# bupt-ai-cz/HIAST

Hardware: AMD Instinct MI355X
Metric: self-training images/sec (fwd+bwd+pseudo-label) at 1024x512 (higher is better)
Workload: dtype fp16

## Files before the change

### hiast_amd/csrc/conv_launch.h

```cpp
#pragma once
#include <stdlib.h>

#include "common.h"

namespace hiast {

struct IGeo {
    int H, W, Ho, Wo, stride, dil;
};

}

struct ConvLaunch {
    const void* x = nullptr;
    const void* wp = nullptr;
    void* y = nullptr;
    const void* res = nullptr;
    const void* res_gate = nullptr;
    int gate_mask = 0;
    const float* gamma = nullptr;
    const float* beta = nullptr;
    const float* mean = nullptr;
    const float* var = nullptr;
    float eps = 0.0f;
    int relu = 0;
    int64_t M = 0;
    int K = 0, N = 0, taps = 1;
    hiast::IGeo geo = {0, 0, 0, 0, 1, 1};
    int fmt = HIAST_FMT_BF16;
    int out_f32 = 0;
    float* stats = nullptr;
    int stats_rows = 0;
    int stats_mode = 0;
    hipStream_t st = nullptr;

    int planes() const { return hiast_fmt_planes(fmt); }
    bool f16() const { return fmt == HIAST_FMT_FP16; }
};

enum class ConvFamily { XCONV, XCONV2, TILE_F16, TILE };

struct ConvRoute {
    ConvFamily family = ConvFamily::TILE;
    int BN = 0, BM = 0;
    bool half9 = false;
    int rows = 0;
};

static inline int conv_panel_streams(int64_t M, int NG, int panel_rows)
{
    static const int env_cus = [] { const char* e = getenv("HIAST_XCONV_CUS"); const int v = e ? atoi(e) : 0; return v >= 8 && v <= 256 ? v : 0; }();
    const long long npanel = (M + panel_rows - 1) / panel_rows;
    long long streams = (env_cus ? env_cus : hiast_grid_cus()) / NG / 8 * 8;
    if (streams < 8) streams = 8;
    if (streams > npanel) streams = (npanel + 7) / 8 * 8;
    return (int)streams;
}

ConvRoute ig_route(const ConvLaunch& c);
int hiast_igemm_launch(const ConvLaunch& c);
int hiast_igemm_launch_f16(const ConvLaunch& c, const ConvRoute& r);
int hiast_xconv_ok(const ConvLaunch& c);
int hiast_xconv_stats_rows(int64_t M, int N);
int hiast_xconv_launch(const ConvLaunch& c, const ConvRoute& r);
int hiast_xconv2_ok(const ConvLaunch& c);
int hiast_xconv2_launch(const ConvLaunch& c);
int hiast_gemm_nt_launch(const void* x, const float* w, void* y, int64_t M, int K, int N, int dtype, hipStream_t st);
```

### hiast_amd/csrc/igemm.hip

```cpp
#include "igemm_kernel.h"

namespace hiast {

template <int PL>
__device__ __forceinline__ size_t ig_wp_elem(int n, int t, int k, int taps, int KO)
{
    const size_t row = ((size_t)n * taps + t) * PL * KO;
    return PL == 2 ? row + (size_t)(k >> 5) * 64 + (k & 31) : row + k;
}

template <int PL, bool F16 = false>
__global__ __launch_bounds__(256) void pack_conv_weight_kernel(const float* __restrict__ w,
                                                               unsigned short* __restrict__ wp,
                                                               unsigned short* __restrict__ wpt, int N, int K, int taps,
                                                               int mode)
{
    const long long idx = (long long)blockIdx.x * 256 + threadIdx.x;
    if (idx >= (long long)N * taps * K) return;
    const int k = (int)(idx % K);
    const int t = (int)((idx / K) % taps);
    const int n = (int)(idx / ((long long)K * taps));
    const float v = w[((size_t)n * K + k) * taps + t];
    unsigned short h, l = 0;
    if (F16) h = H16<true>::enc(v);
    else ig_split(v, h, l);
    if (mode != 1) {
        unsigned short* d = wp + ig_wp_elem<PL>(n, t, k, taps, K);
        d[0] = h;
        if (PL == 2) d[32] = l;
    }
    if (mode != 0) {
        unsigned short* d = (mode == 1 ? wp : wpt) + ig_wp_elem<PL>(k, taps - 1 - t, n, taps, N);
        d[0] = h;
        if (PL == 2) d[32] = l;
    }
}

constexpr int PK_PITCH = 72;

template <int PL, bool F16 = false>
__device__ __forceinline__ void pack_tile(const float* __restrict__ w, unsigned short* __restrict__ wp,
                                          unsigned short* __restrict__ wpt, int N, int K, int taps, int mode, int n0,
                                          int k0, unsigned short* lds)
{
    constexpr int TN = PL == 1 ? 32 : 16;
    unsigned short* hi = lds;
    unsigned short* lo = lds + (PL == 2 ? TN * taps * PK_PITCH : 0);
    unsigned short* fwd = (mode == 1) ? nullptr : wp;
    unsigned short* adj = (mode == 0) ? nullptr : (mode == 1 ? wp : wpt);
    const int run = 64 * taps;
    for (int nh = 0; nh < 64; nh += TN) {
        if (nh) __syncthreads();
        for (int e = threadIdx.x; e < TN * run; e += 256) {
            const int n = e / run, r = e - n * run;
            const int k = r / taps, t = r - k * taps;
            const float v = w[((size_t)(n0 + nh + n) * K + k0) * taps + r];
            unsigned short h, l = 0;
            if (F16) h = H16<true>::enc(v);
            else ig_split(v, h, l);
            hi[(n * taps + t) * PK_PITCH + k] = h;
            if (PL == 2) lo[(n * taps + t) * PK_PITCH + k] = l;
        }
        __syncthreads();
        if (fwd) {
            for (int e = threadIdx.x; e < TN * taps * 8; e += 256) {
                const int c = e & 7, nt = e >> 3;
                const int n = nt / taps, t = nt - n * taps;
                const uint4 vh = *reinterpret_cast<const uint4*>(&hi[nt * PK_PITCH + c * 8]);
                unsigned short* d = fwd + ig_wp_elem<PL>(n0 + nh + n, t, k0 + c * 8, taps, K);
                *reinterpret_cast<uint4*>(d) = vh;
                if (PL == 2) *reinterpret_cast<uint4*>(d + 32) = *reinterpret_cast<const uint4*>(&lo[nt * PK_PITCH + c * 8]);
            }
        }
        if (adj) {
            for (int e = threadIdx.x; e < 64 * taps * (TN / 8); e += 256) {
                const int c = e % (TN / 8), kt = e / (TN / 8);
                const int k = kt / taps, t = kt - k * taps;
                unsigned short vh[8], vl[8];
#pragma unroll
                for (int j = 0; j < 8; ++j) {
                    vh[j] = hi[((c * 8 + j) * taps + t) * PK_PITCH + k];
                    if (PL == 2) vl[j] = lo[((c * 8 + j) * taps + t) * PK_PITCH + k];
                }
                unsigned short* d = adj + ig_wp_elem<PL>(k0 + k, taps - 1 - t, n0 + nh + c * 8, taps, N);
                *reinterpret_cast<uint4*>(d) = make_uint4(vh[0] | (unsigned)vh[1] << 16, vh[2] | (unsigned)vh[3] << 16,
                                                          vh[4] | (unsigned)vh[5] << 16, vh[6] | (unsigned)vh[7] << 16);
                if (PL == 2)
                    *reinterpret_cast<uint4*>(d + 32) = make_uint4(vl[0] | (unsigned)vl[1] << 16, vl[2] | (unsigned)vl[3] << 16,
                                                                   vl[4] | (unsigned)vl[5] << 16, vl[6] | (unsigned)vl[7] << 16);
            }
        }
    }
}

template <int PL, bool F16 = false>
__global__ __launch_bounds__(256) void pack_conv_weight_tiled_kernel(const float* __restrict__ w,
                                                                     unsigned short* __restrict__ wp,
                                                                     unsigned short* __restrict__ wpt, int N, int K,
                                                                     int taps, int mode)
{
    extern __shared__ __attribute__((aligned(16))) unsigned short lds[];
    const int kt = K / 64;
    pack_tile<PL, F16>(w, wp, wpt, N, K, taps, mode, (int)(blockIdx.x / kt) * 64, (int)(blockIdx.x % kt) * 64, lds);
}

__global__ __launch_bounds__(256) void pack_conv_weight_multi_kernel(const hiast_pack_rec* __restrict__ table,
                                                                     const int32_t* __restrict__ chunk_tensor,
                                                                     const int64_t* __restrict__ chunk_start)
{
    extern __shared__ __attribute__((aligned(16))) unsigned short lds[];
    const hiast_pack_rec r = table[chunk_tensor[blockIdx.x]];
    const int kt = r.K / 64;
    const int tile = (int)chunk_start[blockIdx.x];
    const int n0 = (tile / kt) * 64, k0 = (tile % kt) * 64;
    if (r.planes == HIAST_FMT_SPLIT_BF16)
        pack_tile<2>(r.w, (unsigned short*)r.wp, (unsigned short*)r.wpt, r.N, r.K, r.taps, r.mode, n0, k0, lds);
    else if (r.planes == HIAST_FMT_FP16)
        pack_tile<1, true>(r.w, (unsigned short*)r.wp, (unsigned short*)r.wpt, r.N, r.K, r.taps, r.mode, n0, k0, lds);
    else
        pack_tile<1>(r.w, (unsigned short*)r.wp, (unsigned short*)r.wpt, r.N, r.K, r.taps, r.mode, n0, k0, lds);
}

__global__ __launch_bounds__(256) void to_planes_kernel(const float* __restrict__ x, unsigned short* __restrict__ p,
                                                        long long M, int C)
{
    const long long total8 = M * C / 8;
    for (long long i = (long long)blockIdx.x * 256 + threadIdx.x; i < total8; i += (long long)gridDim.x * 256) {
        const long long m = (i * 8) / C;
        const int c = (int)((i * 8) - m * C);
        const float4 a = reinterpret_cast<const float4*>(x)[2 * i], b = reinterpret_cast<const float4*>(x)[2 * i + 1];
        const float v[8] = {a.x, a.y, a.z, a.w, b.x, b.y, b.z, b.w};
        unsigned ph[4], pl_[4];
#pragma unroll
        for (int q = 0; q < 4; ++q) {
            unsigned short h0, l0, h1, l1;
            ig_split(v[2 * q], h0, l0);
            ig_split(v[2 * q + 1], h1, l1);
            ph[q] = (unsigned)h0 | ((unsigned)h1 << 16);
            pl_[q] = (unsigned)l0 | ((unsigned)l1 << 16);
        }
        unsigned short* dst = p + ig_elem<2>((size_t)m, c, C);
        *reinterpret_cast<uint4*>(dst) = make_uint4(ph[0], ph[1], ph[2], ph[3]);
        *reinterpret_cast<uint4*>(dst + 32) = make_uint4(pl_[0], pl_[1], pl_[2], pl_[3]);
    }
}

__global__ __launch_bounds__(256) void from_planes_kernel(const unsigned short* __restrict__ p, float* __restrict__ x,
                                                          long long M, int C)
{
    const long long total8 = M * C / 8;
    for (long long i = (long long)blockIdx.x * 256 + threadIdx.x; i < total8; i += (long long)gridDim.x * 256) {
        const long long m = (i * 8) / C;
        const int c = (int)((i * 8) - m * C);
        const unsigned short* src = p + ig_elem<2>((size_t)m, c, C);
        const uint4 h = *reinterpret_cast<const uint4*>(src), l = *reinterpret_cast<const uint4*>(src + 32);
        const unsigned wh[4] = {h.x, h.y, h.z, h.w}, wl[4] = {l.x, l.y, l.z, l.w};
        float v[8];
#pragma unroll
        for (int q = 0; q < 4; ++q) {
            v[2 * q] = __uint_as_float(wh[q] << 16) + __uint_as_float(wl[q] << 16);
            v[2 * q + 1] = __uint_as_float(wh[q] & 0xFFFF0000u) + __uint_as_float(wl[q] & 0xFFFF0000u);
        }
        reinterpret_cast<float4*>(x)[2 * i] = make_float4(v[0], v[1], v[2], v[3]);
        reinterpret_cast<float4*>(x)[2 * i + 1] = make_float4(v[4], v[5], v[6], v[7]);
    }
}

}

struct IgEnv {
    int half;
    int bn;
    int ragged_off;
    int cosched0;
};
static const IgEnv& ig_env()
{
    static const IgEnv env = [] {
        IgEnv e;
        const char* v = getenv("HIAST_IGEMM_HALF");
        e.half = v ? (atoi(v) != 0) : -1;
        v = getenv("HIAST_IGEMM_BN");
        const int bn = v ? atoi(v) : 0;
        e.bn = (bn == 64 || bn == 128 || bn == 256) ? bn : 0;
        e.ragged_off = getenv("HIAST_IGEMM_RAGGED") != nullptr;
        v = getenv("HIAST_IGEMM_COSCHED");
        e.cosched0 = v && atoi(v) != 0;
        return e;
    }();
    return env;
}
static thread_local int ig_cosched_tls = -1, ig_half_tls = -1;
extern "C" int hiast_igemm_set_half(int v)
{
    const int prev = ig_half_tls;
    ig_half_tls = v < 0 ? -1 : (v != 0);
    return prev;
}
extern "C" int hiast_igemm_set_cosched(int on)
{
    const int prev = ig_cosched_tls;
    ig_cosched_tls = on < 0 ? -1 : (on != 0);
    return prev;
}
static int ig_half_forced() { return ig_half_tls >= 0 ? ig_half_tls : ig_env().half; }
static int ig_cosched() { return ig_cosched_tls >= 0 ? ig_cosched_tls : ig_env().cosched0; }

#ifndef IG_HALF_AUTO
#define IG_HALF_BLOCKS(M, N) ((((M) + 255) / 256) * (((N) % 256 == 0) ? (N) / 256 : (N) / 128))
#define IG_HALF_AUTO(M, K, N) (IG_HALF_BLOCKS(M, N) <= 64 || (IG_HALF_BLOCKS(M, N) <= 128 && !ig_cosched()))
#endif
static int ig_half_tile(int64_t M, int K, int N, int taps, int out_f32)
{
    if (taps != 1 || out_f32 || N % 128 != 0 || M < 4096) return 0;
    if (ig_half_forced() >= 0) return ig_half_forced();
    return IG_HALF_AUTO(M, K, N);
}
static int ig_half_tile9(int64_t M, int N, int PL, bool bn_relu_only)
{
    if (PL != 2 || !bn_relu_only || N % 128 != 0 || M < 4096) return 0;
    if (ig_half_forced() >= 0) return ig_half_forced();
    return IG_HALF_AUTO(M, 0, N);
}

ConvRoute ig_route(const ConvLaunch& c)
{
    ConvRoute r;
    if (c.stats_mode != 2 && hiast_xconv_ok(c)) {
        r.family = ConvFamily::XCONV;
        r.rows = hiast_xconv_stats_rows(c.M, c.N);
        return r;
    }
    if (c.stats_mode == 0 && !c.f16() && hiast_xconv2_ok(c)) {
        r.family = ConvFamily::XCONV2;
        return r;
    }
    r.family = c.f16() ? ConvFamily::TILE_F16 : ConvFamily::TILE;
    r.BN = (c.N % 256 == 0) ? 256 : ((c.N % 128 == 0) ? 128 : 64);
    const bool plain = !c.mean && !c.gamma && !c.res && !c.relu && !c.res_gate && c.stats_mode == 0;
    if (plain && !c.out_f32 && r.BN == 128 && c.N > 512 && !ig_env().ragged_off) r.BN = 256;
    if (const int v = ig_env().bn) {
        if (c.N % v == 0) r.BN = v;
    }
    r.half9 = c.taps == 9 && !c.out_f32 && c.geo.stride == 1 &&
              ig_half_tile9(c.M, c.N, c.planes(), c.mean && c.relu && !c.res && !c.res_gate && c.stats_mode == 0) != 0;
    const bool half = r.half9 || (c.geo.stride >= 0 && ig_half_tile(c.M, c.K, c.N, c.taps, c.out_f32) != 0);
    if (half) r.BN = 128;
    r.BM = half ? 128 : hiast::IG_BM;
    r.rows = (int)((c.M + r.BM - 1) / r.BM);
    return r;
}

int hiast_igemm_launch(const ConvLaunch& in)
{
    ConvLaunch c = in;
    if (c.stats_mode != 2) c.stats_mode = c.stats ? 1 : 0;
    const int H = c.geo.H, W = c.geo.W, stride = c.geo.stride, dil = c.geo.dil;
    if (!hiast_fmt_ok(c.fmt)) return HIAST_E_RANGE;
    const int planes = c.planes();
    if (c.stats_mode == 2) {
        if (!c.stats || !c.res || !c.mean || !c.var || planes != 1 || c.out_f32 || c.relu || c.res_gate || c.N % 8) return HIAST_E_RANGE;
    } else {
        if (c.stats && (planes != 1 || c.out_f32 || c.res || c.relu)) return HIAST_E_RANGE;
        if ((c.stats || c.res_gate) && c.mean) return HIAST_E_RANGE;
    }
    if (c.res_gate && (planes != 1 || !c.res || c.relu || c.out_f32 || (!c.gate_mask && (((uintptr_t)c.res_gate) & 15)))) return HIAST_E_RANGE;
    if (!c.x || !c.wp || !c.y || (c.mean && !c.var)) return HIAST_E_ARG;
    if (c.M <= 0 || c.K <= 0 || c.N <= 0) return HIAST_E_ARG;
    if ((planes != 1 && planes != 2) || (c.taps != 1 && c.taps != 9)) return HIAST_E_RANGE;
    if ((c.K * planes) % 64 != 0 || c.N % 64 != 0 || c.M > (1ll << 31) - 512) return HIAST_E_RANGE;
    if (c.out_f32 && c.res) return HIAST_E_RANGE;
    if ((((uintptr_t)c.x) | ((uintptr_t)c.wp) | ((uintptr_t)c.y) | ((uintptr_t)c.res)) & 15) return HIAST_E_RANGE;
    c.geo = {0, 0, 0, 0, 1, 1};
    size_t in_pix = (size_t)c.M;
    if (c.taps != 1 && stride == -2) {
        if (H <= 0 || W <= 0 || dil != 1 || planes != 1 || c.out_f32) return HIAST_E_ARG;
        const int Hs = (H - 1) / 2 + 1, Ws = (W - 1) / 2 + 1;
        if (c.M % ((int64_t)H * W) != 0) return HIAST_E_ARG;
        c.geo = {Hs, Ws, H, W, -2, 1};
        in_pix = (size_t)(c.M / ((int64_t)H * W)) * Hs * Ws;
    } else if (c.taps != 1) {
        if (H <= 0 || W <= 0 || stride <= 0 || dil <= 0) return HIAST_E_ARG;
        const int Ho = (H - 1) / stride + 1, Wo = (W - 1) / stride + 1;
        if (c.M % ((int64_t)Ho * Wo) != 0) return HIAST_E_ARG;
        c.geo = {H, W, Ho, Wo, stride, dil};
        in_pix = (size_t)(c.M / ((int64_t)Ho * Wo)) * H * W;
    }
    if (in_pix * planes * c.K * 2 >= (1ull << 31) || (size_t)c.N * c.taps * planes * c.K * 2 >= (1ull << 31)) return HIAST_E_RANGE;
    const ConvRoute r = ig_route(c);
    if (c.stats_mode != 0 && c.stats_rows != r.rows) return HIAST_E_ARG;
    switch (r.family) {
    case ConvFamily::XCONV: return hiast_xconv_launch(c, r);
    case ConvFamily::XCONV2: return hiast_xconv2_launch(c);
    case ConvFamily::TILE_F16: return hiast_igemm_launch_f16(c, r);
    case ConvFamily::TILE: break;
    }
    if (planes == 2) return c.out_f32 ? launch_igemm_t<2, true>(c, r) : launch_igemm_t<2, false>(c, r);
    return c.out_f32 ? launch_igemm_t<1, true>(c, r) : launch_igemm_t<1, false>(c, r);
}

extern "C" int hiast_igemm_dgrad_bn_stats(const void* dy, const void* wpt, void* da, int B, int H, int W, int Cin, int Cout,
                                          int taps, int dil, const void* bn_x, const float* gamma, const float* beta,
                                          const float* save_mean, const float* save_invstd, float* partial, int partial_rows,
                                          int fmt, hiast_stream_t stream)
{
    if (fmt != HIAST_FMT_BF16 && fmt != HIAST_FMT_FP16) return HIAST_E_RANGE;
    if (B <= 0 || H <= 0 || W <= 0) return HIAST_E_ARG;
    if (!bn_x || !save_mean || !save_invstd || !partial) return HIAST_E_ARG;
    if ((((uintptr_t)save_mean) | ((uintptr_t)save_invstd) | ((uintptr_t)gamma) | ((uintptr_t)beta)) & 15) return HIAST_E_RANGE;
    ConvLaunch c;
    c.x = dy; c.wp = wpt; c.y = da; c.res = bn_x;
    c.gamma = gamma; c.beta = beta; c.mean = save_mean; c.var = save_invstd;
    c.M = (int64_t)B * H * W; c.K = Cin; c.N = Cout; c.taps = taps;
    c.geo.H = H; c.geo.W = W; c.geo.dil = dil;
    c.fmt = fmt;
    c.stats = partial; c.stats_rows = partial_rows; c.stats_mode = 2;
    c.st = (hipStream_t)stream;
    return hiast_igemm_launch(c);
}

extern "C" int hiast_igemm_dgrad_s2(const void* dy, const void* wpt, void* dx, int B, int H, int W, int Cin, int Cout, int fmt,
                                    hiast_stream_t stream)
{
    if (fmt != HIAST_FMT_BF16 && fmt != HIAST_FMT_FP16) return HIAST_E_RANGE;
    if (B <= 0 || H <= 0 || W <= 0) return HIAST_E_ARG;
    ConvLaunch c;
    c.x = dy; c.wp = wpt; c.y = dx;
    c.M = (int64_t)B * H * W; c.K = Cout; c.N = Cin; c.taps = 9;
    c.geo.H = H; c.geo.W = W; c.geo.stride = -2;
    c.fmt = fmt;
    c.st = (hipStream_t)stream;
    return hiast_igemm_launch(c);
}

extern "C" int hiast_igemm_bn_act(const void* x, const void* wp, const float* gamma, const float* beta,
                                  const float* mean, const float* var, float eps, const void* res, int relu, void* y,
                                  int B, int H, int W, int Cin, int Cout, int taps, int stride, int dil, int fmt,
                                  int out_f32, float* stats, int stats_rows, const void* res_gate, int gate_mask,
                                  hiast_stream_t stream)
{
    if (B <= 0 || H <= 0 || W <= 0) return HIAST_E_ARG;
    if (taps == 1 && stride != 1) return HIAST_E_RANGE;
    const int Ho = taps == 1 ? H : (H - 1) / stride + 1, Wo = taps == 1 ? W : (W - 1) / stride + 1;
    ConvLaunch c;
    c.x = x; c.wp = wp; c.y = y; c.res = res; c.res_gate = res_gate; c.gate_mask = gate_mask;
    c.gamma = gamma; c.beta = beta; c.mean = mean; c.var = var; c.eps = eps;
    c.relu = relu;
    c.M = (int64_t)B * Ho * Wo; c.K = Cin; c.N = Cout; c.taps = taps;
    c.geo.H = H; c.geo.W = W; c.geo.stride = stride; c.geo.dil = dil;
    c.fmt = fmt; c.out_f32 = out_f32;
    c.stats = stats; c.stats_rows = stats_rows;
    c.st = (hipStream_t)stream;
    return hiast_igemm_launch(c);
}

extern "C" int hiast_igemm_stats_rows(int64_t M, int Cin, int Cout, int taps, int fmt)
{
    if (M <= 0 || Cin <= 0 || Cout <= 0) return 0;
    ConvLaunch c;
    c.M = M; c.K = Cin; c.N = Cout; c.taps = taps; c.fmt = fmt;
    c.stats_mode = 1;
    return ig_route(c).rows;
}
extern "C" int hiast_igemm_dgrad_bn_stats_rows(int64_t M, int Cin, int Cout, int taps)
{
    if (M <= 0) return 0;
    ConvLaunch c;
    c.M = M; c.K = Cin; c.N = Cout; c.taps = taps;
    c.stats_mode = 2;
    return ig_route(c).rows;
}

#ifdef IG_STAMP
namespace hiast {
__global__ void ig_stamp_copy_kernel(unsigned* dst)
{
    for (int i = blockIdx.x * blockDim.x + threadIdx.x; i < 1024 * 8 * 8 + 32 * 64; i += gridDim.x * blockDim.x) dst[i] = ig_stamp_buf[i];
}
}
extern "C" int hiast_igemm_debug_stamps(unsigned* dst_device)
{
    hipLaunchKernelGGL(hiast::ig_stamp_copy_kernel, dim3(64), dim3(256), 0, 0, dst_device);
    return (int)hipDeviceSynchronize();
}
#endif

extern "C" int hiast_pack_conv_weight(const float* w, int N, int K, int taps, int fmt, int transpose, void* wp,
                                      void* wpt, hiast_stream_t stream)
{
    if (!w || !wp) return HIAST_E_ARG;
    if (N <= 0 || K <= 0 || taps <= 0) return HIAST_E_ARG;
    const int planes = fmt;
    if (!hiast_fmt_ok(fmt) || transpose < 0 || transpose > 2) return HIAST_E_RANGE;
    if (transpose == 2 && !wpt) return HIAST_E_ARG;
    const long long total = (long long)N * K * taps;
    if (N % 64 == 0 && K % 64 == 0 && taps <= 9 && !((((uintptr_t)wp) | ((uintptr_t)wpt)) & 15)) {
        const dim3 tg((unsigned)((N / 64) * (K / 64)));
        const size_t lds_bytes = (size_t)32 * taps * hiast::PK_PITCH * sizeof(unsigned short);
        if (planes == HIAST_FMT_SPLIT_BF16)
            hipLaunchKernelGGL(hiast::pack_conv_weight_tiled_kernel<2>, tg, dim3(256), lds_bytes, (hipStream_t)stream, w,
                               (unsigned short*)wp, (unsigned short*)wpt, N, K, taps, transpose);
        else if (planes == HIAST_FMT_FP16)
            hipLaunchKernelGGL((hiast::pack_conv_weight_tiled_kernel<1, true>), tg, dim3(256), lds_bytes, (hipStream_t)stream, w,
                               (unsigned short*)wp, (unsigned short*)wpt, N, K, taps, transpose);
        else
            hipLaunchKernelGGL(hiast::pack_conv_weight_tiled_kernel<1>, tg, dim3(256), lds_bytes, (hipStream_t)stream, w,
                               (unsigned short*)wp, (unsigned short*)wpt, N, K, taps, transpose);
        HIAST_CHECK_LAUNCH();
        return 0;
    }
    const dim3 grid((unsigned)((total + 255) / 256));
    if (planes == HIAST_FMT_SPLIT_BF16)
        hipLaunchKernelGGL(hiast::pack_conv_weight_kernel<2>, grid, dim3(256), 0, (hipStream_t)stream, w,
                           (unsigned short*)wp, (unsigned short*)wpt, N, K, taps, transpose);
    else if (planes == HIAST_FMT_FP16)
        hipLaunchKernelGGL((hiast::pack_conv_weight_kernel<1, true>), grid, dim3(256), 0, (hipStream_t)stream, w,
                           (unsigned short*)wp, (unsigned short*)wpt, N, K, taps, transpose);
    else
        hipLaunchKernelGGL(hiast::pack_conv_weight_kernel<1>, grid, dim3(256), 0, (hipStream_t)stream, w,
                           (unsigned short*)wp, (unsigned short*)wpt, N, K, taps, transpose);
    HIAST_CHECK_LAUNCH();
    return 0;
}

namespace hiast {

template <int INK, int PL, bool F16 = false>
__global__ __launch_bounds__(256) void stem_tail_kernel(const void* __restrict__ xv, const float* __restrict__ gamma,
                                                        const float* __restrict__ beta, const float* __restrict__ mean,
                                                        const float* __restrict__ var, float eps,
                                                        unsigned short* __restrict__ out, int B, int H, int W, int C, int Ho,
                                                        int Wo)
{
    const int G = C >> 3;
    const long long total = (long long)B * Ho * Wo * G;
    const long long stride = (long long)gridDim.x * 256;
    long long i = (long long)blockIdx.x * 256 + threadIdx.x;
    if (i >= total) return;
    const int cg = (int)(i % G);
    float sc[8], sh[8];
#pragma unroll
    for (int k = 0; k < 8; ++k) {
        const int c = cg * 8 + k;
        const float invstd = 1.0f / sqrtf(var[c] + eps);
        sc[k] = (gamma ? gamma[c] : 1.0f) * invstd;
        sh[k] = fmaf(-mean[c], sc[k], beta ? beta[c] : 0.0f);
    }
    for (; i < total; i += stride) {
        const long long pix = i / G;
        const int xo = (int)(pix % Wo);
        const int yo = (int)((pix / Wo) % Ho);
        const int b = (int)(pix / ((long long)Wo * Ho));
        float m[8];
#pragma unroll
        for (int k = 0; k < 8; ++k) m[k] = -INFINITY;
#pragma unroll
        for (int dy = 0; dy < 3; ++dy) {
            const int yy = 2 * yo - 1 + dy;
            if (yy < 0 || yy >= H) continue;
#pragma unroll
            for (int dx = 0; dx < 3; ++dx) {
                const int xx = 2 * xo - 1 + dx;
                if (xx < 0 || xx >= W) continue;
                const size_t off = (((size_t)b * H + yy) * W + xx) * C + cg * 8;
                float v[8];
                if (INK != 0) {
                    const uint4 r = *reinterpret_cast<const uint4*>(reinterpret_cast<const unsigned short*>(xv) + off);
                    const unsigned w4[4] = {r.x, r.y, r.z, r.w};
#pragma unroll
                    for (int q = 0; q < 4; ++q) {
                        v[2 * q] = H16<INK == 2>::lo(w4[q]);
                        v[2 * q + 1] = H16<INK == 2>::hi(w4[q]);
                    }
                } else {
                    const float4 a = *reinterpret_cast<const float4*>(reinterpret_cast<const float*>(xv) + off);
                    const float4 c4 = *reinterpret_cast<const float4*>(reinterpret_cast<const float*>(xv) + off + 4);
                    v[0] = a.x; v[1] = a.y; v[2] = a.z; v[3] = a.w; v[4] = c4.x; v[5] = c4.y; v[6] = c4.z; v[7] = c4.w;
                }
#pragma unroll
                for (int k = 0; k < 8; ++k) {
                    float t = fmaf(v[k], sc[k], sh[k]);
                    t = t > 0.f ? t : 0.f;
                    if (INK != 0) t = H16<INK == 2>::dec(H16<INK == 2>::enc(t));
                    m[k] = t > m[k] ? t : m[k];
                }
            }
        }
        unsigned ph[4], pl_[4];
#pragma unroll
        for (int q = 0; q < 4; ++q) {
            unsigned short h0, l0 = 0, h1, l1 = 0;
            if (PL == 2) {
                ig_split(m[2 * q], h0, l0);
                ig_split(m[2 * q + 1], h1, l1);
            } else {
                h0 = H16<F16>::enc(m[2 * q]);
                h1 = H16<F16>::enc(m[2 * q + 1]);
            }
            ph[q] = (unsigned)h0 | ((unsigned)h1 << 16);
            pl_[q] = (unsigned)l0 | ((unsigned)l1 << 16);
        }
        unsigned short* dst = out + ig_elem<PL>((size_t)pix, cg * 8, C);
        *reinterpret_cast<uint4*>(dst) = make_uint4(ph[0], ph[1], ph[2], ph[3]);
        if (PL == 2) *reinterpret_cast<uint4*>(dst + 32) = make_uint4(pl_[0], pl_[1], pl_[2], pl_[3]);
    }
}

}

extern "C" int hiast_stem_tail(const void* x, int dtype, const float* gamma, const float* beta, const float* mean,
                               const float* var, float eps, void* out, int fmt, int B, int H, int W, int C,
                               hiast_stream_t stream)
{
    if (!hiast_fmt_ok(fmt)) return HIAST_E_RANGE;
    const int planes = hiast_fmt_planes(fmt), f16 = fmt == HIAST_FMT_FP16;
    if (!x || !mean || !var || !out) return HIAST_E_ARG;
    if (B <= 0 || H <= 0 || W <= 0 || C <= 0) return HIAST_E_ARG;
    if (dtype < 0 || dtype > 2 || C % 8 != 0 || (planes == 2 && C % 32 != 0) ||
        ((((uintptr_t)x) | ((uintptr_t)out)) & 15))
        return HIAST_E_RANGE;
    const int Ho = (H - 1) / 2 + 1, Wo = (W - 1) / 2 + 1, G = C / 8;
    const long long total = (long long)B * Ho * Wo * G;
    if ((long long)B * H * W * C >= (1ll << 40)) return HIAST_E_RANGE;
    long long nb = (total + 255) / 256;
    int grid = (int)(nb > 16384 ? 16384 : nb);
    {
        long long a = 256, g = G;
        while (a) { const long long t = g % a; g = a; a = t; }
        const int need = (int)(G / g);
        if (grid >= need) grid -= grid % need;
        else return HIAST_E_RANGE;
    }
    hipStream_t st = (hipStream_t)stream;
#define L(BF, PL)                                                                                                  \
    hipLaunchKernelGGL((hiast::stem_tail_kernel<BF, PL>), dim3(grid), dim3(256), 0, st, x, gamma, beta, mean, var, eps, \
                       (unsigned short*)out, B, H, W, C, Ho, Wo)
#define LF(BF)                                                                                                     \
    hipLaunchKernelGGL((hiast::stem_tail_kernel<BF, 1, true>), dim3(grid), dim3(256), 0, st, x, gamma, beta, mean, var, eps, \
                       (unsigned short*)out, B, H, W, C, Ho, Wo)
    if (f16) { if (dtype == 2) LF(2); else if (dtype == 1) LF(1); else LF(0); }
    else if (dtype == 2) { if (planes == 2) L(2, 2); else L(2, 1); }
    else if (dtype == 1) { if (planes == 2) L(1, 2); else L(1, 1); }
    else { if (planes == 2) L(0, 2); else L(0, 1); }
#undef LF
#undef L
    HIAST_CHECK_LAUNCH();
    return 0;
}

extern "C" int hiast_split_planes(float* x, void* planes, int64_t M, int C, int inverse, hiast_stream_t stream)
{
    if (!x || !planes) return HIAST_E_ARG;
    if (M <= 0 || C <= 0) return HIAST_E_ARG;
    if (C % 32 != 0 || ((((uintptr_t)x) | ((uintptr_t)planes)) & 15)) return HIAST_E_RANGE;
    const long long total8 = (long long)M * C / 8;
    long long nb = (total8 + 255) / 256;
    const int grid = (int)(nb < 1 ? 1 : (nb > 8192 ? 8192 : nb));
    if (inverse)
        hipLaunchKernelGGL(hiast::from_planes_kernel, dim3(grid), dim3(256), 0, (hipStream_t)stream,
                           (const unsigned short*)planes, x, (long long)M, C);
    else
        hipLaunchKernelGGL(hiast::to_planes_kernel, dim3(grid), dim3(256), 0, (hipStream_t)stream, (const float*)x,
                           (unsigned short*)planes, (long long)M, C);
    HIAST_CHECK_LAUNCH();
    return 0;
}

extern "C" int hiast_pack_conv_weight_multi(const hiast_pack_rec* table, const int32_t* chunk_tensor,
                                            const int64_t* chunk_start, int n_chunks, int max_taps, hiast_stream_t stream)
{
    if (!table || !chunk_tensor || !chunk_start) return HIAST_E_ARG;
    if (n_chunks <= 0 || max_taps <= 0) return HIAST_E_ARG;
    if (max_taps > 9) return HIAST_E_RANGE;
    const size_t lds_bytes = (size_t)32 * max_taps * hiast::PK_PITCH * sizeof(unsigned short);
    hipLaunchKernelGGL(hiast::pack_conv_weight_multi_kernel, dim3(n_chunks), dim3(256), lds_bytes, (hipStream_t)stream, table,
                       chunk_tensor, chunk_start);
    HIAST_CHECK_LAUNCH();
    return 0;
}
```

### hiast_amd/csrc/xconv.hip

```cpp
#include <hip/hip_bf16.h>
#include <stdlib.h>

#include "conv_launch.h"

namespace hiast {

constexpr int XC_PANEL = 64;
constexpr int XC_STAGES = 3;
constexpr int XC_COLS = 512;

__device__ __forceinline__ h_bf16x8 xc_lds_read(unsigned addr)
{
    h_bf16x8 v;
    asm volatile("ds_read_b128 %0, %1" : "=v"(v) : "v"(addr));
    return v;
}
__device__ __forceinline__ void xc_lds_wait(h_bf16x8& a, h_bf16x8& b)
{
    asm volatile("s_waitcnt lgkmcnt(0)" : "+v"(a), "+v"(b));
}

__device__ __forceinline__ int xc_chan(int g, int b, int r) { return (b >> 1) * 32 + g * 8 + (b & 1) * 4 + r; }

template <int KC, bool BN, bool RES, bool RELU, bool GATE, bool STATS, bool F16 = false>
__global__ __launch_bounds__(512) void xconv_kernel(const unsigned short* __restrict__ X,
                                                    const unsigned short* __restrict__ Wp,
                                                    const float* __restrict__ gamma, const float* __restrict__ beta,
                                                    const float* __restrict__ mean, const float* __restrict__ var,
                                                    float eps, const unsigned short* __restrict__ R,
                                                    const unsigned char* __restrict__ Rg,
                                                    unsigned short* __restrict__ Y, int M, int N,
                                                    float* __restrict__ stats)
{
    constexpr int SL = KC / 64;
    constexpr int KS = KC / 32;
    constexpr int STAGE = XC_PANEL * KC * 2;
    __shared__ __attribute__((aligned(1024))) unsigned char smem[XC_STAGES * STAGE];
    __shared__ float s_sc[XC_COLS], s_sh[XC_COLS];

    const int tid = threadIdx.x, lane = tid & 63;
    const int wave = __builtin_amdgcn_readfirstlane(tid >> 6);
    const int g = lane >> 4, px = lane & 15;
    const int NG = N / XC_COLS;
    const int xcd = blockIdx.x & 7, slot = blockIdx.x >> 3;
    const int cg = slot % NG;
    const int nstream = (int)gridDim.x / NG;
    const int stream = (slot / NG) * 8 + xcd;
    const int n0 = cg * XC_COLS + wave * 64;
    const int npanel = (M + XC_PANEL - 1) / XC_PANEL;

    h_bf16x8 wr[4][KS];
#pragma unroll
    for (int b = 0; b < 4; ++b) {
        const unsigned short* wrow = Wp + (size_t)(n0 + xc_chan(px >> 2, b, px & 3)) * KC + g * 8;
#pragma unroll
        for (int s = 0; s < KS; ++s) wr[b][s] = *reinterpret_cast<const h_bf16x8*>(wrow + s * 32);
    }
#pragma unroll
    for (int b = 0; b < 4; ++b)
#pragma unroll
        for (int s = 0; s < KS; ++s) asm volatile("" : "+v"(wr[b][s]));
    if (BN) {
        for (int c = tid; c < XC_COLS; c += 512) {
            const int n = cg * XC_COLS + c;
            const float sc = (gamma ? gamma[n] : 1.0f) * (1.0f / sqrtf(var[n] + eps));
            s_sc[c] = sc;
            s_sh[c] = fmaf(-mean[n], sc, beta ? beta[n] : 0.0f);
        }
        __syncthreads();
    }

    constexpr int OOB = (int)0x80000000;
    const __amdgpu_buffer_rsrc_t xrs = __builtin_amdgcn_make_buffer_rsrc((void*)X, 0, (int)((size_t)M * KC * 2), 0x00020000);
    const int drow = wave * 8 + (lane >> 3);
    const int dchunk = ((lane & 7) ^ ((drow >> 1) & 7)) * 16;
    auto issue = [&](int p, int st) {
        const int m = p * XC_PANEL + drow;
        const int voff = (p < npanel && m < M) ? (int)((size_t)m * KC * 2) + dchunk : OOB;
        unsigned char* base = smem + st * STAGE + wave * 1024;
#pragma unroll
        for (int j = 0; j < SL; ++j) h_dma16(xrs, base + j * (XC_PANEL * 128), voff, j * 128);
    };

    const unsigned lds_base = (unsigned)(size_t)smem;
    float st1[STATS ? 16 : 1], st2[STATS ? 16 : 1];
#pragma unroll
    for (int q = 0; q < (STATS ? 16 : 1); ++q) { st1[q] = 0.f; st2[q] = 0.f; }

    issue(stream, 0);
    issue(stream + nstream, 1);
    int it = 0;
    for (int p = stream; p < npanel; p += nstream, ++it) {
        const int st = it % XC_STAGES;
        constexpr int NRES = RES ? (GATE ? 8 : 4) : 0;
        if (it == 0) asm volatile("s_waitcnt vmcnt(%0)\n\ts_barrier" ::"n"(SL) : "memory");
        else asm volatile("s_waitcnt vmcnt(%0)\n\ts_barrier" ::"n"(SL + 8 + NRES) : "memory");
        uint4 rres[RES ? 2 : 1][2];
        unsigned rgate[GATE ? 2 : 1][2];
        auto load_res = [&](int half) {
#pragma unroll
            for (int t = 0; t < 2; ++t) {
                const int m = p * XC_PANEL + half * 32 + t * 16 + px;
                const size_t row = (size_t)(m < M ? m : 0) * N + n0 + g * 8;
                rres[t][0] = h_load16_once(R + row);
                rres[t][1] = h_load16_once(R + row + 32);
                if (GATE) {
                    const unsigned char* gp = Rg + (size_t)(m < M ? m : 0) * (N >> 3) + ((n0 + g * 8) >> 3);
                    rgate[t][0] = gp[0];
                    rgate[t][1] = gp[4];
                }
            }
        };
        if (RES) load_res(0);
        issue(p + 2 * nstream, (it + 2) % XC_STAGES);
#pragma unroll
        for (int half = 0; half < 2; ++half) {
            if (RES && half == 1) load_res(1);
            h_f32x4 acc[2][4];
#pragma unroll
            for (int a = 0; a < 2; ++a)
#pragma unroll
                for (int b = 0; b < 4; ++b) acc[a][b] = (h_f32x4){0.f, 0.f, 0.f, 0.f};
            auto frag = [&](int s, int a) {
                return xc_lds_read(lds_base + (unsigned)(st * STAGE + (s >> 1) * (XC_PANEL * 128) +
                                                         h_lds_off(half * 32 + a * 16 + px, (s & 1) * 4 + g)));
            };
            constexpr bool DB = !(STATS || (BN && RES));
            h_bf16x8 xa[DB ? 2 : 1][2];
            xa[0][0] = frag(0, 0);
            xa[0][1] = frag(0, 1);
            xc_lds_wait(xa[0][0], xa[0][1]);
#pragma unroll
            for (int s = 0; s < KS; ++s) {
                constexpr int one = DB ? 1 : 0;
                if (DB && s + 1 < KS) {
                    xa[(s + 1) & one][0] = frag(s + 1, 0);
                    xa[(s + 1) & one][1] = frag(s + 1, 1);
                }
#pragma unroll
                for (int a = 0; a < 2; ++a)
#pragma unroll
                    for (int b = 0; b < 4; ++b)
                        acc[a][b] = H16<F16>::mfma16(wr[b][s], xa[s & one][a], acc[a][b]);
                if (s + 1 < KS) {
                    if (!DB) {
                        xa[0][0] = frag(s + 1, 0);
                        xa[0][1] = frag(s + 1, 1);
                    }
                    xc_lds_wait(xa[(s + 1) & one][0], xa[(s + 1) & one][1]);
                }
            }
#pragma unroll
            for (int a = 0; a < 2; ++a) {
                const int m = p * XC_PANEL + half * 32 + a * 16 + px;
                const bool ok = m < M;
                const size_t row = (size_t)(ok ? m : 0) * N + n0 + g * 8;
                const uint4 r0 = rres[RES ? a : 0][0], r1 = rres[RES ? a : 0][1];
                const unsigned gate0 = GATE ? rgate[GATE ? a : 0][0] : 0xFFu;
                const unsigned gate1 = GATE ? rgate[GATE ? a : 0][1] : 0xFFu;
                float o[16];
#pragma unroll
                for (int b = 0; b < 4; ++b)
#pragma unroll
                    for (int r = 0; r < 4; ++r) o[(b >> 1) * 8 + (b & 1) * 4 + r] = acc[a][b][r];
                if (BN) {
#pragma unroll
                    for (int hh = 0; hh < 2; ++hh) {
                        const int c = wave * 64 + hh * 32 + g * 8;
#pragma unroll
                        for (int q = 0; q < 8; q += 4) {
                            const float4 sc = *reinterpret_cast<const float4*>(&s_sc[c + q]);
                            const float4 sh = *reinterpret_cast<const float4*>(&s_sh[c + q]);
                            o[hh * 8 + q] = fmaf(o[hh * 8 + q], sc.x, sh.x);
                            o[hh * 8 + q + 1] = fmaf(o[hh * 8 + q + 1], sc.y, sh.y);
                            o[hh * 8 + q + 2] = fmaf(o[hh * 8 + q + 2], sc.z, sh.z);
                            o[hh * 8 + q + 3] = fmaf(o[hh * 8 + q + 3], sc.w, sh.w);
                        }
                    }
                }
                if (RES) {
                    const unsigned w0[4] = {r0.x, r0.y, r0.z, r0.w}, w1[4] = {r1.x, r1.y, r1.z, r1.w};
#pragma unroll
                    for (int q = 0; q < 4; ++q) {
                        float a0 = H16<F16>::lo(w0[q]), a1 = H16<F16>::hi(w0[q]);
                        float b0 = H16<F16>::lo(w1[q]), b1 = H16<F16>::hi(w1[q]);
                        if (GATE) {
                            a0 = ((gate0 >> (2 * q)) & 1u) ? a0 : 0.f;
                            a1 = ((gate0 >> (2 * q + 1)) & 1u) ? a1 : 0.f;
                            b0 = ((gate1 >> (2 * q)) & 1u) ? b0 : 0.f;
                            b1 = ((gate1 >> (2 * q + 1)) & 1u) ? b1 : 0.f;
                        }
                        o[2 * q] += a0;
                        o[2 * q + 1] += a1;
                        o[8 + 2 * q] += b0;
                        o[8 + 2 * q + 1] += b1;
                    }
                }
                if (RELU) {
#pragma unroll
                    for (int q = 0; q < 16; ++q) o[q] = o[q] > 0.f ? o[q] : 0.f;
                }
                unsigned pk[8];
                if (STATS && F16) {
#pragma unroll
                    for (int q = 0; q < 8; ++q) {
                        pk[q] = H16<F16>::pack(o[2 * q], o[2 * q + 1]);
                        if (ok) {
                            const float v0 = H16<F16>::lo(pk[q]), v1 = H16<F16>::hi(pk[q]);
                            st1[2 * q] += v0; st2[2 * q] = fmaf(v0, v0, st2[2 * q]);
                            st1[2 * q + 1] += v1; st2[2 * q + 1] = fmaf(v1, v1, st2[2 * q + 1]);
                        }
                        __builtin_amdgcn_sched_barrier(0);
                    }
                } else {
#pragma unroll
                    for (int q = 0; q < 8; ++q) pk[q] = H16<F16>::pack(o[2 * q], o[2 * q + 1]);
                    if (STATS && ok) {
#pragma unroll
                        for (int q = 0; q < 8; ++q) {
                            const float v0 = H16<F16>::lo(pk[q]), v1 = H16<F16>::hi(pk[q]);
                            st1[2 * q] += v0; st2[2 * q] = fmaf(v0, v0, st2[2 * q]);
                            st1[2 * q + 1] += v1; st2[2 * q + 1] = fmaf(v1, v1, st2[2 * q + 1]);
                        }
                    }
                }
                if (ok) {
                    h_store16_out(Y + row, pk[0], pk[1], pk[2], pk[3]);
                    h_store16_out(Y + row + 32, pk[4], pk[5], pk[6], pk[7]);
                }
            }
        }
    }
    if (STATS) {
#pragma unroll
        for (int q = 0; q < 16; ++q) {
#pragma unroll
            for (int o = 1; o < 16; o <<= 1) {
                st1[q] += __shfl_xor(st1[q], o, 64);
                st2[q] += __shfl_xor(st2[q], o, 64);
            }
        }
        if (px == 0) {
            float* d = stats + ((size_t)stream * N + n0 + g * 8) * 2;
#pragma unroll
            for (int q = 0; q < 8; ++q) {
                d[2 * q] = st1[q];
                d[2 * q + 1] = st2[q];
                d[64 + 2 * q] = st1[8 + q];
                d[64 + 2 * q + 1] = st2[8 + q];
            }
        }
    }
}

}

int hiast_xconv_ok(const ConvLaunch& c)
{
    const char* env = getenv("HIAST_XCONV");
    const bool has_bn = c.mean != nullptr, has_res = c.res != nullptr;
    if ((env && atoi(env) == 0) || c.planes() != 1 || c.taps != 1 || c.out_f32) return 0;
    if (c.K != 256 || c.N % hiast::XC_COLS != 0 || c.N > 2048) return 0;
    if (c.res_gate && (!c.gate_mask || !has_res || c.relu)) return 0;
    if (has_bn && has_res && !c.relu) return 0;
    if (c.stats_mode == 1 && (has_res || c.relu || has_bn)) return 0;
    if (c.M < 4096) return 0;
    return 1;
}

int hiast_xconv_stats_rows(int64_t M, int N)
{
    return conv_panel_streams(M, N / hiast::XC_COLS, hiast::XC_PANEL);
}

int hiast_xconv_launch(const ConvLaunch& c, const ConvRoute& r)
{
    using namespace hiast;
    const dim3 grid((unsigned)(r.rows * (c.N / XC_COLS)));
#define XK(BNF, RESF, RELUF, GATEF, STATSF, F16)                                                                      \
    hipLaunchKernelGGL((xconv_kernel<256, BNF, RESF, RELUF, GATEF, STATSF, F16>), grid, dim3(512), 0, c.st,           \
                       (const unsigned short*)c.x, (const unsigned short*)c.wp, c.gamma, c.beta, c.mean, c.var, c.eps, \
                       (const unsigned short*)c.res, (const unsigned char*)c.res_gate, (unsigned short*)c.y, (int)c.M, c.N, \
                       c.stats)
#define XL(BNF, RESF, RELUF, GATEF, STATSF)                                                                          \
    do {                                                                                                             \
        if (c.f16()) XK(BNF, RESF, RELUF, GATEF, STATSF, true);                                                      \
        else XK(BNF, RESF, RELUF, GATEF, STATSF, false);                                                             \
    } while (0)
    const bool bn = c.mean != nullptr;
    if (c.stats) { XL(false, false, false, false, true); }
    else if (c.res_gate) { XL(false, true, false, true, false); }
    else if (c.res) {
        if (bn) { if (c.relu) XL(true, true, true, false, false); else return HIAST_E_RANGE; }
        else { if (c.relu) XL(false, true, true, false, false); else XL(false, true, false, false, false); }
    } else {
        if (bn) { if (c.relu) XL(true, false, true, false, false); else XL(true, false, false, false, false); }
        else { if (c.relu) XL(false, false, true, false, false); else XL(false, false, false, false, false); }
    }
#undef XL
#undef XK
    HIAST_CHECK_LAUNCH();
    return 0;
}
```

Measured before the change: 141.6.

## Add weight-stationary streaming 1x1 conv kernel for K=512

Adds a specialised 1x1 conv kernel for K=512 that keeps each wave's weight slice in registers, streams 32-row input panels through a 3-stage LDS pipeline via buffer DMA, and fuses BN, residual, gate, ReLU and stats epilogues. The router now sends K=512 convs that meet a minimum-work threshold to this kernel instead of the generic tiled igemm path. The aim is to raise the MFMA-to-memory ratio for these layers. The cost is heavy register pressure from the resident weights, and the work threshold means it only applies to large shapes.

```diff
diff --git a/hiast_amd/csrc/conv_launch.h b/hiast_amd/csrc/conv_launch.h
--- a/hiast_amd/csrc/conv_launch.h
+++ b/hiast_amd/csrc/conv_launch.h
@@ -61,8 +61,11 @@
 int hiast_igemm_launch(const ConvLaunch& c);
 int hiast_igemm_launch_f16(const ConvLaunch& c, const ConvRoute& r);
 int hiast_xconv_ok(const ConvLaunch& c);
-int hiast_xconv_stats_rows(int64_t M, int N);
+int hiast_xconv_stats_rows(int64_t M, int K, int N);
 int hiast_xconv_launch(const ConvLaunch& c, const ConvRoute& r);
+int hiast_xconv512_ok(const ConvLaunch& c);
+int hiast_xconv512_stats_rows(int64_t M, int N);
+int hiast_xconv512_launch(const ConvLaunch& c, const ConvRoute& r);
 int hiast_xconv2_ok(const ConvLaunch& c);
 int hiast_xconv2_launch(const ConvLaunch& c);
 int hiast_gemm_nt_launch(const void* x, const float* w, void* y, int64_t M, int K, int N, int dtype, hipStream_t st);
diff --git a/hiast_amd/csrc/igemm.hip b/hiast_amd/csrc/igemm.hip
--- a/hiast_amd/csrc/igemm.hip
+++ b/hiast_amd/csrc/igemm.hip
@@ -228,7 +228,7 @@
     ConvRoute r;
     if (c.stats_mode != 2 && hiast_xconv_ok(c)) {
         r.family = ConvFamily::XCONV;
-        r.rows = hiast_xconv_stats_rows(c.M, c.N);
+        r.rows = hiast_xconv_stats_rows(c.M, c.K, c.N);
         return r;
     }
     if (c.stats_mode == 0 && !c.f16() && hiast_xconv2_ok(c)) {
diff --git a/hiast_amd/csrc/xconv.hip b/hiast_amd/csrc/xconv.hip
--- a/hiast_amd/csrc/xconv.hip
+++ b/hiast_amd/csrc/xconv.hip
@@ -260,22 +260,25 @@
     const char* env = getenv("HIAST_XCONV");
     const bool has_bn = c.mean != nullptr, has_res = c.res != nullptr;
     if ((env && atoi(env) == 0) || c.planes() != 1 || c.taps != 1 || c.out_f32) return 0;
+    if (c.M < 4096) return 0;
+    if (c.K == 512) return hiast_xconv512_ok(c);
     if (c.K != 256 || c.N % hiast::XC_COLS != 0 || c.N > 2048) return 0;
     if (c.res_gate && (!c.gate_mask || !has_res || c.relu)) return 0;
     if (has_bn && has_res && !c.relu) return 0;
     if (c.stats_mode == 1 && (has_res || c.relu || has_bn)) return 0;
-    if (c.M < 4096) return 0;
     return 1;
 }
 
-int hiast_xconv_stats_rows(int64_t M, int N)
-{
+int hiast_xconv_stats_rows(int64_t M, int K, int N)
+{
+    if (K == 512) return hiast_xconv512_stats_rows(M, N);
     return conv_panel_streams(M, N / hiast::XC_COLS, hiast::XC_PANEL);
 }
 
 int hiast_xconv_launch(const ConvLaunch& c, const ConvRoute& r)
 {
     using namespace hiast;
+    if (c.K == 512) return hiast_xconv512_launch(c, r);
     const dim3 grid((unsigned)(r.rows * (c.N / XC_COLS)));
 #define XK(BNF, RESF, RELUF, GATEF, STATSF, F16)                                                                      \
     hipLaunchKernelGGL((xconv_kernel<256, BNF, RESF, RELUF, GATEF, STATSF, F16>), grid, dim3(512), 0, c.st,           \
diff --git a/hiast_amd/csrc/xconv512.hip b/hiast_amd/csrc/xconv512.hip
--- /dev/null
+++ b/hiast_amd/csrc/xconv512.hip
@@ -0,0 +1,296 @@
+#include <hip/hip_bf16.h>
+#include <stdlib.h>
+
+#include "conv_launch.h"
+
+namespace hiast {
+
+constexpr int X5_PANEL = 32;
+constexpr int X5_STAGES = 3;
+constexpr int X5_COLS = 256;
+constexpr int X5_K = 512;
+constexpr int X5_ROWB = X5_K * 2;
+constexpr int X5_STAGE = X5_PANEL * X5_ROWB;
+
+template <int IDX>
+__device__ __forceinline__ h_bf16x8 x5_lds_read_i(unsigned addr)
+{
+    h_bf16x8 v;
+    asm volatile("ds_read_b128 %0, %1 offset:%2" : "=v"(v) : "v"(addr), "i"(IDX * 2048));
+    return v;
+}
+__device__ __forceinline__ h_bf16x8 x5_lds_read(unsigned addr, int idx)
+{
+    switch (idx) {
+    case 1: return x5_lds_read_i<1>(addr);
+    case 2: return x5_lds_read_i<2>(addr);
+    case 3: return x5_lds_read_i<3>(addr);
+    case 4: return x5_lds_read_i<4>(addr);
+    case 5: return x5_lds_read_i<5>(addr);
+    case 6: return x5_lds_read_i<6>(addr);
+    case 7: return x5_lds_read_i<7>(addr);
+    case 8: return x5_lds_read_i<8>(addr);
+    case 9: return x5_lds_read_i<9>(addr);
+    case 10: return x5_lds_read_i<10>(addr);
+    case 11: return x5_lds_read_i<11>(addr);
+    case 12: return x5_lds_read_i<12>(addr);
+    case 13: return x5_lds_read_i<13>(addr);
+    case 14: return x5_lds_read_i<14>(addr);
+    case 15: return x5_lds_read_i<15>(addr);
+    default: return x5_lds_read_i<0>(addr);
+    }
+}
+__device__ __forceinline__ void x5_lds_wait(h_bf16x8& a, h_bf16x8& b)
+{
+    asm volatile("s_waitcnt lgkmcnt(0)" : "+v"(a), "+v"(b));
+}
+
+template <bool BN, bool RES, bool RELU, bool GATE, bool STATS, bool F16>
+__global__ __launch_bounds__(512) void xconv512_kernel(const unsigned short* __restrict__ X,
+                                                       const unsigned short* __restrict__ Wp,
+                                                       const float* __restrict__ gamma, const float* __restrict__ beta,
+                                                       const float* __restrict__ mean, const float* __restrict__ var,
+                                                       float eps, const unsigned short* __restrict__ R,
+                                                       const unsigned char* __restrict__ Rg,
+                                                       unsigned short* __restrict__ Y, int M, int N,
+                                                       float* __restrict__ stats)
+{
+    constexpr int KS = X5_K / 32;
+    __shared__ __attribute__((aligned(1024))) unsigned char smem[X5_STAGES * X5_STAGE];
+
+    const int tid = threadIdx.x, lane = tid & 63;
+    const int wave = __builtin_amdgcn_readfirstlane(tid >> 6);
+    const int g = lane >> 4, px = lane & 15;
+    const int NG = N / X5_COLS;
+    const int xcd = blockIdx.x & 7, slot = blockIdx.x >> 3;
+    const int cg = slot % NG;
+    const int nstream = (int)gridDim.x / NG;
+    const int stream = (slot / NG) * 8 + xcd;
+    const int n0 = cg * X5_COLS + wave * 32;
+    const int npanel = (M + X5_PANEL - 1) / X5_PANEL;
+    const int c0 = n0 + g * 8;
+
+    h_bf16x8 wr[2][KS];
+#pragma unroll
+    for (int b = 0; b < 2; ++b) {
+        const unsigned short* wrow = Wp + (size_t)(n0 + (px >> 2) * 8 + b * 4 + (px & 3)) * X5_K + g * 8;
+#pragma unroll
+        for (int s = 0; s < KS; ++s) wr[b][s] = *reinterpret_cast<const h_bf16x8*>(wrow + s * 32);
+    }
+    float sc[BN ? 8 : 1], sh[BN ? 8 : 1];
+    if (BN) {
+#pragma unroll
+        for (int q = 0; q < 8; ++q) {
+            const int n = c0 + q;
+            sc[q] = (gamma ? gamma[n] : 1.0f) * (1.0f / sqrtf(var[n] + eps));
+            sh[q] = fmaf(-mean[n], sc[q], beta ? beta[n] : 0.0f);
+        }
+    }
+#pragma unroll
+    for (int b = 0; b < 2; ++b)
+#pragma unroll
+        for (int s = 0; s < KS; ++s) asm volatile("" : "+v"(wr[b][s]));
+    if (BN) {
+#pragma unroll
+        for (int q = 0; q < 8; ++q) asm volatile("" : "+v"(sc[q]), "+v"(sh[q]));
+    }
+
+    constexpr int OOB = (int)0x80000000;
+    const __amdgpu_buffer_rsrc_t xrs = __builtin_amdgcn_make_buffer_rsrc((void*)X, 0, (int)((size_t)M * X5_ROWB), 0x00020000);
+    const int rgrp = wave & 3, j0 = (wave >> 2) * 4;
+    const int drow = rgrp * 8 + (lane >> 3);
+    const int dchunk = ((lane & 7) ^ ((drow >> 1) & 7)) * 16;
+    auto issue = [&](int p, int st) {
+        const int m = p * X5_PANEL + drow;
+        const int voff = (p < npanel && m < M) ? (int)((size_t)m * X5_ROWB) + dchunk : OOB;
+        unsigned char* base = smem + st * X5_STAGE + rgrp * 1024;
+#pragma unroll
+        for (int j = 0; j < 4; ++j) h_dma16(xrs, base + (j0 + j) * (X5_PANEL * 128), voff, (j0 + j) * 128);
+    };
+    const unsigned lds_base = (unsigned)(size_t)smem;
+
+    float st1[STATS ? 8 : 1], st2[STATS ? 8 : 1];
+#pragma unroll
+    for (int q = 0; q < (STATS ? 8 : 1); ++q) { st1[q] = 0.f; st2[q] = 0.f; }
+
+    constexpr int NRES = RES ? (GATE ? 4 : 2) : 0;
+    struct Rows {
+        uint4 res[2];
+        unsigned char gate[2];
+    };
+    Rows ring[2];
+    auto load_rows = [&](Rows& r, int p) {
+        if (!RES) return;
+#pragma unroll
+        for (int a = 0; a < 2; ++a) {
+            const int m = p * X5_PANEL + a * 16 + px;
+            const size_t mr = (size_t)((p < npanel && m < M) ? m : 0);
+            r.res[a] = h_load16_once(R + mr * N + c0);
+            if (GATE) r.gate[a] = Rg[mr * (N >> 3) + (c0 >> 3)];
+        }
+    };
+
+    auto panel = [&](int p, int it, const Rows& cur, Rows& nxt) {
+        const int st = it % X5_STAGES;
+        asm volatile("s_waitcnt vmcnt(%0)\n\ts_barrier" ::"n"(6 + NRES) : "memory");
+        load_rows(nxt, p + nstream);
+        issue(p + 2 * nstream, (it + 2) % X5_STAGES);
+
+        h_f32x4 acc[2][2];
+#pragma unroll
+        for (int a = 0; a < 2; ++a)
+#pragma unroll
+            for (int b = 0; b < 2; ++b) acc[a][b] = (h_f32x4){0.f, 0.f, 0.f, 0.f};
+        const unsigned fbase = lds_base + (unsigned)(st * X5_STAGE) + (unsigned)h_lds_off(px, g);
+        auto frag = [&](int s, int a) { return x5_lds_read((s & 1) ? fbase ^ 64u : fbase, 2 * (s >> 1) + a); };
+        h_bf16x8 xa[2][2];
+        xa[0][0] = frag(0, 0);
+        xa[0][1] = frag(0, 1);
+        x5_lds_wait(xa[0][0], xa[0][1]);
+#pragma unroll
+        for (int s = 0; s < KS; ++s) {
+            if (s + 1 < KS) {
+                xa[(s + 1) & 1][0] = frag(s + 1, 0);
+                xa[(s + 1) & 1][1] = frag(s + 1, 1);
+            }
+#pragma unroll
+            for (int a = 0; a < 2; ++a)
+#pragma unroll
+                for (int b = 0; b < 2; ++b) acc[a][b] = H16<F16>::mfma16(wr[b][s], xa[s & 1][a], acc[a][b]);
+            if (s + 1 < KS) x5_lds_wait(xa[(s + 1) & 1][0], xa[(s + 1) & 1][1]);
+        }
+        __builtin_amdgcn_sched_barrier(0);
+#pragma unroll
+        for (int a = 0; a < 2; ++a) {
+            const int m = p * X5_PANEL + a * 16 + px;
+            const bool ok = m < M;
+            float o[8];
+#pragma unroll
+            for (int b = 0; b < 2; ++b)
+#pragma unroll
+                for (int r = 0; r < 4; ++r) o[b * 4 + r] = acc[a][b][r];
+            if (BN) {
+#pragma unroll
+                for (int q = 0; q < 8; ++q) o[q] = fmaf(o[q], sc[q], sh[q]);
+            }
+            if (RES) {
+                const unsigned w0[4] = {cur.res[a].x, cur.res[a].y, cur.res[a].z, cur.res[a].w};
+                const unsigned gate = GATE ? cur.gate[a] : 0xFFu;
+#pragma unroll
+                for (int q = 0; q < 4; ++q) {
+                    float r0 = H16<F16>::lo(w0[q]), r1 = H16<F16>::hi(w0[q]);
+                    if (GATE) {
+                        r0 = ((gate >> (2 * q)) & 1u) ? r0 : 0.f;
+                        r1 = ((gate >> (2 * q + 1)) & 1u) ? r1 : 0.f;
+                    }
+                    o[2 * q] += r0;
+                    o[2 * q + 1] += r1;
+                }
+            }
+            if (RELU) {
+#pragma unroll
+                for (int q = 0; q < 8; ++q) o[q] = o[q] > 0.f ? o[q] : 0.f;
+            }
+            unsigned pk[4];
+#pragma unroll
+            for (int q = 0; q < 4; ++q) pk[q] = H16<F16>::pack(o[2 * q], o[2 * q + 1]);
+            asm volatile("" : "+v"(pk[0]), "+v"(pk[1]), "+v"(pk[2]), "+v"(pk[3]));
+            if (STATS && ok) {
+#pragma unroll
+                for (int q = 0; q < 4; ++q) {
+                    const float v0 = H16<F16>::lo(pk[q]), v1 = H16<F16>::hi(pk[q]);
+                    st1[2 * q] += v0; st2[2 * q] = fmaf(v0, v0, st2[2 * q]);
+                    st1[2 * q + 1] += v1; st2[2 * q + 1] = fmaf(v1, v1, st2[2 * q + 1]);
+                }
+            }
+            if (ok) h_store16_out(Y + (size_t)m * N + c0, pk[0], pk[1], pk[2], pk[3]);
+        }
+    };
+
+    load_rows(ring[0], stream);
+    issue(stream, 0);
+    issue(stream + nstream, 1);
+    asm volatile("s_waitcnt vmcnt(4)" ::: "memory");
+    int p = stream, it = 0;
+    for (; p + nstream < npanel; p += 2 * nstream, it += 2) {
+        panel(p, it, ring[0], ring[1]);
+        panel(p + nstream, it + 1, ring[1], ring[0]);
+    }
+    if (p < npanel) panel(p, it, ring[0], ring[1]);
+    if (STATS) {
+#pragma unroll
+        for (int q = 0; q < 8; ++q) {
+#pragma unroll
+            for (int o = 1; o < 16; o <<= 1) {
+                st1[q] += __shfl_xor(st1[q], o, 64);
+                st2[q] += __shfl_xor(st2[q], o, 64);
+            }
+        }
+        if (px == 0) {
+            float* d = stats + ((size_t)stream * N + c0) * 2;
+#pragma unroll
+            for (int q = 0; q < 8; ++q) {
+                d[2 * q] = st1[q];
+                d[2 * q + 1] = st2[q];
+            }
+        }
+    }
+}
+
+enum { X5_PLAIN = 1, X5_STATS = 2, X5_BN_RES_RELU = 4, X5_GATED = 8, X5_ANY_SHAPE = 16 };
+constexpr int X5_DEFAULT_MASK = X5_PLAIN | X5_STATS | X5_BN_RES_RELU | X5_GATED;
+
+static int x5_variant(const ConvLaunch& c)
+{
+    const bool has_bn = c.mean != nullptr, has_res = c.res != nullptr;
+    if (c.stats_mode == 1) return (has_bn || has_res || c.relu || c.res_gate) ? 0 : X5_STATS;
+    if (c.res_gate) return (c.gate_mask && has_res && !c.relu && !has_bn) ? X5_GATED : 0;
+    if (has_bn && has_res && c.relu) return X5_BN_RES_RELU;
+    if (!has_bn && !c.gamma && !has_res && !c.relu) return X5_PLAIN;
+    return 0;
+}
+
+}
+
+int hiast_xconv512_ok(const ConvLaunch& c)
+{
+    const char* env = getenv("HIAST_XCONV512");
+    const int mask = env ? atoi(env) : hiast::X5_DEFAULT_MASK;
+    if (c.K != hiast::X5_K || c.N % hiast::X5_COLS != 0 || c.N > 2048 || c.stats_mode == 2) return 0;
+    const int v = hiast::x5_variant(c);
+    const int rounds = (v & (hiast::X5_BN_RES_RELU | hiast::X5_GATED)) ? 4 : 8;
+    if (!(mask & hiast::X5_ANY_SHAPE) && ((c.M + 255) / 256) * (c.N / 256) < (long long)rounds * hiast_grid_cus()) return 0;
+    return (v & mask) != 0;
+}
+
+int hiast_xconv512_stats_rows(int64_t M, int N)
+{
+    return conv_panel_streams(M, N / hiast::X5_COLS, hiast::X5_PANEL);
+}
+
+int hiast_xconv512_launch(const ConvLaunch& c, const ConvRoute& r)
+{
+    using namespace hiast;
+    const dim3 grid((unsigned)(r.rows * (c.N / X5_COLS)));
+#define XK(BNF, RESF, RELUF, GATEF, STATSF, F16)                                                                      \
+    hipLaunchKernelGGL((xconv512_kernel<BNF, RESF, RELUF, GATEF, STATSF, F16>), grid, dim3(512), 0, c.st,             \
+                       (const unsigned short*)c.x, (const unsigned short*)c.wp, c.gamma, c.beta, c.mean, c.var, c.eps, \
+                       (const unsigned short*)c.res, (const unsigned char*)c.res_gate, (unsigned short*)c.y, (int)c.M, c.N, \
+                       c.stats)
+#define XL(BNF, RESF, RELUF, GATEF, STATSF)                                                                          \
+    do {                                                                                                             \
+        if (c.f16()) XK(BNF, RESF, RELUF, GATEF, STATSF, true);                                                      \
+        else XK(BNF, RESF, RELUF, GATEF, STATSF, false);                                                             \
+    } while (0)
+    switch (x5_variant(c)) {
+    case X5_STATS: XL(false, false, false, false, true); break;
+    case X5_GATED: XL(false, true, false, true, false); break;
+    case X5_BN_RES_RELU: XL(true, true, true, false, false); break;
+    case X5_PLAIN: XL(false, false, false, false, false); break;
+    default: return HIAST_E_RANGE;
+    }
+#undef XL
+#undef XK
+    HIAST_CHECK_LAUNCH();
+    return 0;
+}
```

After: 141.9 (median of 2 runs). About the same (+0.2%).
